# limix/CellRegMap

Measured on AMD Instinct MI355X. Metric: variant-tests/sec (interaction test), higher is better.
Workload: dtype f64

## Files before the change

cellregmap_amd/_lib.py:

```python
import ctypes
import os

import numpy as np

_HERE = os.path.dirname(os.path.abspath(__file__))
LIB_PATH = os.path.join(_HERE, "libcrm_hip.so")

c_double_p = ctypes.POINTER(ctypes.c_double)
c_int_p = ctypes.POINTER(ctypes.c_int)
c_long_p = ctypes.POINTER(ctypes.c_long)
vp = ctypes.c_void_p

SIGNATURES = {
    "crm_last_error": (ctypes.c_char_p, []),
    "crm_version": (ctypes.c_char_p, []),
    "crm_ctx_create": (ctypes.c_int, [ctypes.c_int, ctypes.POINTER(vp)]),
    "crm_ctx_destroy": (None, [vp]),
    "crm_ctx_synchronize": (ctypes.c_int, [vp]),
    "crm_ctx_trim": (ctypes.c_int, [vp]),
    "crm_background_create_qs": (ctypes.c_int, [vp, ctypes.c_long, ctypes.c_int, vp, vp, vp, vp,
                                                ctypes.POINTER(vp)]),
    "crm_background_create": (ctypes.c_int, [vp, ctypes.c_long, vp, ctypes.c_int, vp, ctypes.c_long,
                                             ctypes.c_int, vp, ctypes.c_double, ctypes.POINTER(vp)]),
    "crm_background_create_hadamard": (ctypes.c_int, [vp, ctypes.c_long, vp, ctypes.c_int, vp, ctypes.c_int, vp,
# ... 28 lines not shown
    "crm_panel_destroy": (None, [vp]),
    "crm_scan_interaction": (ctypes.c_int, [vp, vp, ctypes.c_long, ctypes.c_long] + [vp] * 13),
    "crm_scan_interaction_info": (ctypes.c_int, [vp, vp, ctypes.c_long, ctypes.c_long] + [vp] * 6),
    "crm_scan_interaction_bounds": (ctypes.c_int, [vp, vp, ctypes.c_long, ctypes.c_long] + [vp] * 8),
    "crm_scan_interaction_permuted": (ctypes.c_int, [vp, vp, ctypes.c_long, ctypes.c_long, ctypes.c_int] + [vp] * 8),
    "crm_scan_interaction_multi": (ctypes.c_int, [vp, ctypes.c_int, vp, ctypes.c_long, ctypes.c_long] + [vp] * 8),
    "crm_scan_interaction_tail": (ctypes.c_int, [vp, vp, ctypes.c_long, ctypes.c_long] + [vp] * 15),
    "crm_scan_interaction_permuted_tail": (ctypes.c_int, [vp, vp, ctypes.c_long, ctypes.c_long, ctypes.c_int] + [vp] * 10),
    "crm_scan_interaction_multi_tail": (ctypes.c_int, [vp, ctypes.c_int, vp, ctypes.c_long, ctypes.c_long] + [vp] * 10),
    "crm_scan_association": (ctypes.c_int, [vp, vp, ctypes.c_long, ctypes.c_long, ctypes.c_int, vp, vp, vp]),
    "crm_association_null_multi": (ctypes.c_int, [vp, ctypes.c_int, vp]),
    "crm_scan_association_multi": (ctypes.c_int, [vp, ctypes.c_int, vp, ctypes.c_long, ctypes.c_long, ctypes.c_int, vp, vp,
                                                  vp]),
    "crm_lmm_fit": (ctypes.c_int, [vp, ctypes.c_int, vp, vp]),
    "crm_cov_solve": (ctypes.c_int, [vp, ctypes.c_int, ctypes.c_double, ctypes.c_double, vp, ctypes.c_int, vp]),
    "crm_effects_multi": (ctypes.c_int, [vp, vp, ctypes.c_long, vp, ctypes.c_int, vp, ctypes.c_int, vp, ctypes.c_int, vp,
                                         ctypes.c_int, vp, ctypes.c_int, ctypes.c_int, vp, vp, vp, vp]),
    "crm_set_block_variants": (ctypes.c_int, [vp, ctypes.c_int]),
    "crm_set_null_fit_polish": (ctypes.c_int, [vp, ctypes.c_int]),
    "crm_set_progress_callback": (ctypes.c_int, [vp, vp, vp]),
    "crm_set_fast_rotation": (ctypes.c_int, [vp, ctypes.c_int]),
    "crm_kernel_timer_reset": (ctypes.c_int, [vp]),
    "crm_kernel_timer_read": (ctypes.c_int, [vp, c_double_p, c_long_p, c_double_p, c_double_p]),
    "crm_kernel_timer_stop": (ctypes.c_int, [vp]),
    "crm_test_set_form": (ctypes.c_int, [ctypes.c_char_p, ctypes.c_int, ctypes.c_int]),
    "crm_test_set_contraction": (ctypes.c_int, [vp, ctypes.c_int, ctypes.c_int]),
    "crm_test_set_shared_h": (ctypes.c_int, [vp, ctypes.c_int]),
    "crm_test_tail_launches": (ctypes.c_long, [vp]),
    "crm_test_spectrum_tail_launches": (ctypes.c_long, [vp]),
    "crm_test_dense_repeats": (ctypes.c_long, [vp]),
    "crm_test_donor_pair_blocks": (ctypes.c_long, [vp]),
    "crm_test_unrelated_donor_blocks": (ctypes.c_int, [vp, ctypes.POINTER(ctypes.c_long)]),
    "crm_test_gram_dma_launches": (ctypes.c_int, [vp, ctypes.POINTER(ctypes.c_long)]),
    "crm_test_tests_without_pair": (ctypes.c_long, [vp]),
    "crm_test_set_contraction_sync": (ctypes.c_int, [vp, ctypes.c_int]),
    "crm_test_sync_fallbacks": (ctypes.c_long, [vp]),
    "crm_test_overruns": (ctypes.c_long, []),
    "crm_test_live_device_bytes": (ctypes.c_long, []),
    "crm_test_set_kinship_route": (ctypes.c_int, [vp, ctypes.c_int]),
    "crm_test_check_context": (ctypes.c_int, [vp]),
    "crm_test_overrun_selftest": (ctypes.c_int, [vp]),
    "crm_test_null_fit_probe": (ctypes.c_int, [vp, ctypes.c_int, ctypes.c_double]),
    "crm_test_null_fit_probe_read": (ctypes.c_int, [vp, vp, ctypes.c_long]),
    "crm_test_contract": (ctypes.c_int, [vp, ctypes.c_long, ctypes.c_int, ctypes.c_int, vp, vp, vp,
                                         ctypes.c_int]),
    "crm_test_contract_kr": (ctypes.c_int, [vp, ctypes.c_long, ctypes.c_int, ctypes.c_int, ctypes.c_int,
                                            vp, vp, vp, vp]),
    "crm_test_contract_kr_t": (ctypes.c_int, [vp, ctypes.c_long, ctypes.c_int, ctypes.c_int, ctypes.c_int,
                                              vp, vp, vp, vp]),
    "crm_test_eigh": (ctypes.c_int, [vp, ctypes.c_int, ctypes.c_int, vp, vp, vp, ctypes.c_int, vp, vp]),
    "crm_test_eigh2": (ctypes.c_int, [vp, ctypes.c_int, ctypes.c_int, vp, vp, vp, vp, vp, ctypes.c_int, vp, vp, vp]),
    "crm_test_back_tasks": (ctypes.c_int, [ctypes.c_int, ctypes.c_long, ctypes.c_int, vp, ctypes.c_int, c_int_p]),
    "crm_test_dc_plan": (ctypes.c_int, [vp, vp, ctypes.c_int, ctypes.c_int, ctypes.c_double, c_int_p, c_double_p, vp, vp, vp,
                                        c_int_p, vp]),
    "crm_test_eigvalsh": (ctypes.c_int, [vp, ctypes.c_int, ctypes.c_int, vp, vp]),
    "crm_test_davies": (ctypes.c_int, [vp, ctypes.c_int, ctypes.c_int, vp, vp, vp, vp, vp]),
    "crm_test_tail_pvalue": (ctypes.c_int, [vp, ctypes.c_int, ctypes.c_int, vp, vp, vp, vp, vp]),
}

_lib = None


class CrmError(RuntimeError):
    pass


# ... 30 lines not shown
```

cellregmap_amd/csrc/api_core.hip:

```cpp
#include <dlfcn.h>

#include <algorithm>
#include <atomic>
#include <cstdarg>
#include <mutex>

#include <map>

#include "crm_internal.h"
#include "eigh.h"

namespace crm {

static thread_local std::string g_error;

void set_error(const char* fmt, ...) {
    char buf[1024];
    va_list ap;
    va_start(ap, fmt);
    vsnprintf(buf, sizeof buf, fmt, ap);
    va_end(ap);
    g_error = buf;
}

// ... 235 lines not shown

int crm_set_null_fit_polish(crm_ctx* c, int on) {
    return crm::guarded_on("crm_set_null_fit_polish", c, [&]() -> int {
    if (!c) return CRM_ERR_ARG;
    c->polish = on != 0;
    return CRM_OK;
    });
}

int crm_set_progress_callback(crm_ctx* c, void (*callback)(long, long, void*), void* user) {
    return crm::guarded_on("crm_set_progress_callback", c, [&]() -> int {
    if (!c) return CRM_ERR_ARG;
    if (callback) c->progress[std::this_thread::get_id()] = crm_ctx::Progress{callback, user};
    else c->progress.erase(std::this_thread::get_id());
    return CRM_OK;
    });
}

int crm_set_fast_rotation(crm_ctx* c, int on) {
    return crm::guarded_on("crm_set_fast_rotation", c, [&]() -> int {
    if (!c) return CRM_ERR_ARG;
    c->fast_T = on != 0;
    return CRM_OK;
    });
}

extern "C++" {
namespace crm {
namespace {
struct FormSlot { const char* name; int value; bool set; };
FormSlot g_forms[] = {{"gram_staged", 0, false}, {"kr_no_tail", 0, false}, {"nullfit_per_wave", 0, false}, {"kin_fold", 0, false},
                      {"eigh_one_stage", 0, false}, {"nullfit_exact", 0, false}, {"donor_pairs", 0, false},
                      {"pairs_without_kinship_term", 0, false}, {"flat_kappa_milli", 0, false}, {"chase_abort", 0, false}, {"nullfit_one_per_wave", 0, false},
                      {"kin_diag", 0, false}, {"donor_pairs_rotate", 0, false}};
std::mutex g_forms_mu;
}
int form(const char* name, int otherwise) {
    std::lock_guard<std::mutex> lock(g_forms_mu);
    for (const FormSlot& f : g_forms)
        if (strcmp(f.name, name) == 0) return f.set ? f.value : otherwise;
    return otherwise;
}
}
}

int crm_test_set_form(const char* name, int value, int reset) {
    return crm::guarded("crm_test_set_form", [&]() -> int {
    if (!name) return CRM_ERR_ARG;
    std::lock_guard<std::mutex> lock(crm::g_forms_mu);
    for (crm::FormSlot& f : crm::g_forms)
        if (strcmp(f.name, name) == 0) {
            f.value = value;
            f.set = reset == 0;
            return CRM_OK;
        }
    crm::set_error("crm_test_set_form: no kernel form is called '%s'", name);
    return CRM_ERR_ARG;
    });
}

int crm_kernel_timer_reset(crm_ctx* c) {
    return crm::guarded_on("crm_kernel_timer_reset", c, [&]() -> int {
    if (!c) return CRM_ERR_ARG;
    CRM_HIP(hipSetDevice(c->device));
    CRM_HIP(hipStreamSynchronize(c->stream));
    c->timed_used = 0;
    c->kr_flops = 0.0;
// ... 270 lines not shown
```

cellregmap_amd/csrc/crm_internal.h:

```cpp
#pragma once
#include <map>
#include <mutex>
#include <thread>
#include <type_traits>
#include <utility>

#include "crm_common.h"

namespace crm {

constexpr int CRM_DEFAULT_BLOCK = 1024;
constexpr int CRM_MAX_AUTO_BLOCK = 4096;
constexpr int CRM_MAX_RHO = 16;
constexpr int CRM_MAX_COV = 8;
constexpr int CRM_MAX_COV_WIDE = 62;
constexpr int CRM_MAX_COV_XWIDE = 128;
constexpr int CRM_MAX_K0 = 256;
constexpr int CRM_MAX_GRAM_ROWS = 288;
constexpr int DT_SUMS_LD = 136;
constexpr int BLOCK_SLACK_MAX = 4096;

struct DevBuf {
    void* ptr = nullptr;
    size_t bytes = 0;
// ... 35 lines not shown
struct crm_ctx {
    std::recursive_mutex mu;
    int device = 0;
    hipStream_t stream = nullptr;
    hipStream_t upload_stream = nullptr;
    hipEvent_t ev0 = nullptr, ev1 = nullptr;
    int block_variants = 0;
    bool fast_T = true;
    int kin_route = 1;
    bool fast_gene_rot = true;
    bool collapse = true;
    struct Progress { void (*fn)(long done, long total, void* user) = nullptr; void* user = nullptr; };
    std::map<std::thread::id, Progress> progress;
    bool progress_muted = false;
    void report(long done, long total) {
        if (progress_muted) return;
        auto it = progress.find(std::this_thread::get_id());
        if (it != progress.end() && it->second.fn) it->second.fn(done, total, it->second.user);
    }
    bool in_scan = false;
    bool polish = false;
    bool probe_on = false;
    double probe_x = 0.0;
    std::vector<double> probe_out;
    bool nullfit_exact = false;
    crm::GemmTune tune;
    crm::DevBuf sync_counters;
    unsigned* sync_timeouts_host = nullptr;
    long sync_fallbacks = 0;
    long dense_repeats = 0;
    long tail_launches = 0;
    long spectrum_tail_launches = 0;
    long donor_pair_blocks = 0;
    long unrelated_donor_blocks = 0;
    long gram_dma_launches = 0;
    long tests_without_pair = 0;
    struct ReplayBlock {
        long col0 = 0;
        int nb = 0;
        bool collapsed = false;
        std::vector<char> fit;
        crm::DevBuf T;
    };
    int replay_mode = 0;
    size_t replay_cursor = 0;
    std::vector<ReplayBlock*> replay_blocks;
    void replay_clear() {
        for (ReplayBlock* b : replay_blocks) delete b;
        replay_blocks.clear();
        replay_cursor = 0;
        replay_mode = 0;
    }
    crm::EighWork* eigh_ws = nullptr;
    bool eigh_ws_busy = false;
    bool timing = false;
    std::vector<std::pair<hipEvent_t, hipEvent_t>> timed;
    size_t timed_used = 0;
    double kr_flops = 0.0;
    crm::DevBuf ws_T, ws_A, ws_Gb, ws_Gx, ws_Gs, ws_G2, ws_GG, ws_Gt, ws_Z, ws_small, ws_probs, ws_F, ws_Gext, ws_TH, ws_AH, ws_XG;
    crm::DevBuf ws_xwide;
    crm::DevBuf ws_Tcut;
    crm::DevBuf ws_Gk, ws_S, ws_S2;
    crm::DevBuf ws_WB;
    crm::DevBuf ws_Pd;
    crm::DevBuf ws_Anone;
    std::vector<crm::DevBuf*> all_bufs() {
// ... 18 lines not shown
```

cellregmap_amd/csrc/kinship.hip:

```cpp
#include <algorithm>
#include <atomic>

#include "nullfit.h"
#include "objects.h"

using namespace crm;

namespace crm {

void jacobi_rotate(int k, double* A, double* V, int p, int q, double cs, double sn) {
    for (int r = 0; r < k; r++) {
        const double arp = A[(size_t)r * k + p], arq = A[(size_t)r * k + q];
        A[(size_t)r * k + p] = cs * arp - sn * arq;
        A[(size_t)r * k + q] = sn * arp + cs * arq;
    }
    for (int r = 0; r < k; r++) {
        const double apr = A[(size_t)p * k + r], aqr = A[(size_t)q * k + r];
        A[(size_t)p * k + r] = cs * apr - sn * aqr;
        A[(size_t)q * k + r] = sn * apr + cs * aqr;
    }
    for (int r = 0; r < k; r++) {
        const double vrp = V[(size_t)r * k + p], vrq = V[(size_t)r * k + q];
        V[(size_t)r * k + p] = cs * vrp - sn * vrq;
        V[(size_t)r * k + q] = sn * vrp + cs * vrq;
// ... 35 lines not shown
        for (long e = d + 1; e < groups; e++) {
            double s = 0.0;
            for (long q = 0; q < m; q++) s += hKd[d * m + q] * hKd[e * m + q];
            if (!(std::fabs(s) <= tol * std::sqrt(kappa[d] * kappa[e]))) return CRM_OK;
        }
    crm_ctx* ctx = bg->ctx;
    hipStream_t st = ctx->stream;
    const long ldc = round_up(KK, 128);
    if (sizeof(double) * (double)groups * KK * ldc > (double)(1ull << 30)) return CRM_OK;
    DevBuf dC, probs_dev;
    CRM_TRY(dC.ensure(sizeof(double) * (size_t)groups * KK * ldc));
    std::vector<GemmProblem> pr((size_t)groups);
    long maxlen = GEMM_BK;
    for (long d = 0; d < groups; d++) {
        GemmProblem p{};
        p.X = bg->kin_Y.as<double>() + bg->kin_row0[d] * bg->kin_ldy; p.ldx = bg->kin_ldy;
        p.Y = p.X; p.ldy = bg->kin_ldy;
        p.C = dC.as<double>() + (size_t)d * KK * ldc; p.ldc = ldc;
        p.M = KK; p.N = KK; p.cells = bg->kin_len[d];
        maxlen = std::max(maxlen, bg->kin_len[d]);
        pr[d] = p;
    }
    CRM_TRY(probs_dev.ensure(sizeof(GemmProblem) * pr.size()));
    CRM_HIP(hipMemcpyAsync(probs_dev.ptr, pr.data(), sizeof(GemmProblem) * pr.size(), hipMemcpyHostToDevice, st));
    CRM_TRY(launch_gemm_tn(ctx, probs_dev.as<GemmProblem>(), (int)groups, KK, KK, maxlen, false, 0, 1, 0));
    std::vector<double> C((size_t)groups * KK * ldc);
    CRM_HIP(hipMemcpyAsync(C.data(), dC.ptr, sizeof(double) * C.size(), hipMemcpyDeviceToHost, st));
    CRM_HIP(hipStreamSynchronize(st));
    const int k2pad = (int)round_up(k2, GEMM_BK);
    const long P = groups * k2, ldp = round_up(P, 128);
    std::vector<double> hU((size_t)groups * k2pad * 128, 0.0), hR((size_t)k1 * ldp, 0.0), hEE((size_t)k1 * k1, 0.0),
        lam((size_t)P, 0.0);
    std::vector<double> A((size_t)k2 * k2), V, w;
    for (long d = 0; d < groups; d++) {
        const double* Cd = C.data() + (size_t)d * KK * ldc;
        for (int i = 0; i < k2; i++)
            for (int j = 0; j < k2; j++) A[(size_t)i * k2 + j] = 0.5 * (Cd[i * ldc + j] + Cd[j * ldc + i]);
        jacobi_eigh(k2, A, V, w);
        double wmax = 0.0;
        for (int j = 0; j < k2; j++) wmax = std::max(wmax, w[j]);
        double* Ud = hU.data() + (size_t)d * k2pad * 128;
        for (int j = 0; j < k2; j++) {
            if (!(w[j] > (double)k2 * 2.220446049250313e-16 * wmax)) continue;
            const double sc = 1.0 / std::sqrt(w[j]);
            lam[d * k2 + j] = w[j];
            for (int q = 0; q < k2; q++) Ud[(size_t)q * 128 + j] = V[(size_t)q * k2 + j] * sc;
            for (int a = 0; a < k1; a++) {
                double s = 0.0;
                for (int q = 0; q < k2; q++) s += Ud[(size_t)q * 128 + j] * Cd[q * ldc + k2 + a];
                hR[(size_t)a * ldp + d * k2 + j] = s;
            }
        }
        for (int a = 0; a < k1; a++)
            for (int e = 0; e < k1; e++) hEE[(size_t)a * k1 + e] += Cd[(k2 + a) * ldc + k2 + e];
    }
    CRM_TRY(bg->wb_U.ensure(sizeof(double) * hU.size()));
    CRM_TRY(bg->wb_R.ensure(sizeof(double) * hR.size()));
    CRM_TRY(bg->wb_EE.ensure(sizeof(double) * hEE.size()));
    CRM_HIP(hipMemcpyAsync(bg->wb_U.ptr, hU.data(), sizeof(double) * hU.size(), hipMemcpyHostToDevice, st));
    CRM_HIP(hipMemcpyAsync(bg->wb_R.ptr, hR.data(), sizeof(double) * hR.size(), hipMemcpyHostToDevice, st));
    CRM_HIP(hipMemcpyAsync(bg->wb_EE.ptr, hEE.data(), sizeof(double) * hEE.size(), hipMemcpyHostToDevice, st));
    std::vector<std::vector<double>> s0(bg->nrho, std::vector<double>((size_t)ldp, 0.0));
    for (int i = 0; i < bg->nrho; i++) {
        for (long p = 0; p < P; p++) s0[i][p] = (1.0 - bg->rho[i]) * kappa[p / k2] * lam[p];
        CRM_TRY(bg->wb_S0[i].ensure(sizeof(double) * (size_t)ldp));
        CRM_HIP(hipMemcpyAsync(bg->wb_S0[i].ptr, s0[i].data(), sizeof(double) * (size_t)ldp, hipMemcpyHostToDevice, st));
    }
    CRM_HIP(hipStreamSynchronize(st));
    bg->wb_P = P;
    bg->wb_ldp = ldp;
    bg->wb_k2pad = k2pad;
    static std::atomic<unsigned long> wb_tables_made{0};
    bg->wb_gen = ++wb_tables_made;
    bg->kin_wb = true;
    return CRM_OK;
}

}

extern "C" {

int crm_background_set_kinship_groups(crm_background* bg, const int* group, long groups, const double* hKd, long m,
                                      const double* U, int k2) {
    return crm::guarded_on("crm_background_set_kinship_groups", bg ? bg->ctx : nullptr, [&]() -> int {
    if (!bg || !group || !hKd || !U || groups < 1 || m < 1 || k2 < 1) return CRM_ERR_ARG;
    if (bg->builder) {
        set_error("kinship groups: the background is still under construction");
        return CRM_ERR_ARG;
    }
    const long n = bg->n;
    const int k1 = (int)(bg->cols - (long)k2 * m);
    if (!bg->fast_T || !bg->H.ptr || k1 < 1 || k1 + k2 > 2 * CRM_MAX_K0 || groups > 4096) return CRM_OK;
    for (long i = 0; i < n; i++)
        if (group[i] < 0 || group[i] >= groups) {
            set_error("kinship groups: group index %d at cell %ld outside [0, %ld)", group[i], i, groups);
            return CRM_ERR_ARG;
        }
    crm_ctx* ctx = bg->ctx;
    CRM_HIP(hipSetDevice(ctx->device));
    hipStream_t st = ctx->stream;
    bg->kin = false;
    struct Undo {
// ... 131 lines not shown
```

cellregmap_amd/csrc/objects.h:

```cpp
#pragma once
#include <cmath>
#include <memory>

#include "crm_internal.h"

namespace crm {
constexpr long CELL_PAD = 128;
}

struct crm_donor_tables {
    unsigned long e0_key = 0, group_key = 0;
    unsigned long stamp = 0;
    crm::DevBuf TZ;
    crm::DevBuf Bd;
    crm::DevBuf Z2;
    crm::DevBuf Z3;
};

struct crm_background_builder;

struct crm_background {
    ~crm_background();
    crm_background_builder* builder = nullptr;
    crm_ctx* ctx = nullptr;
    long n = 0, n_pad = 0;
    int nrho = 0;
    double rho[crm::CRM_MAX_RHO] = {0};
    int r[crm::CRM_MAX_RHO] = {0};
    double ortho_defect[crm::CRM_MAX_RHO] = {0};
    long ldq = 0;
    crm::DevBuf Q0[crm::CRM_MAX_RHO];
    bool q0_ready[crm::CRM_MAX_RHO] = {false};
    crm::DevBuf Ht;
    crm::DevBuf S0[crm::CRM_MAX_RHO];
    std::vector<double> s0_max;
    bool fast_T = false;
    long ldh = 0, cols = 0;
    crm::DevBuf H;
    crm::DevBuf Mix[crm::CRM_MAX_RHO];
    bool kin = false;
    long kin_groups = 0, kin_groups_pad = 0;
    long kin_cols = 0;
    int kin_k1 = 0, kin_k2 = 0;
    long kin_rows = 0;
    std::vector<long> kin_row0, kin_len;
    crm::DevBuf kin_map;
    crm::DevBuf kin_Y;
    long kin_ldy = 128;
    crm::DevBuf kin_hKd;
    long kin_ldh = 0;
    bool kin_fold = false;
    long kin_kdim = 0;
    crm::DevBuf MixK[crm::CRM_MAX_RHO];
    bool kin_wb = false;
    long wb_P = 0, wb_ldp = 0;
    int wb_k2pad = 0;
    crm::DevBuf wb_U;
    crm::DevBuf wb_R;
    crm::DevBuf wb_EE;
    crm::DevBuf wb_S0[crm::CRM_MAX_RHO];
    unsigned long wb_gen = 0;
    static constexpr int DT_CACHE = 2;
    std::vector<crm_donor_tables*> dt_cache;
    unsigned long dt_clock = 0;
};

int crm_background_require_q0(crm_background* bg, int i);

struct crm_gene {
    crm_background* bg = nullptr;
    crm_ctx* ctx = nullptr;
    int c = 0, k0 = 0;
    long ld_yw = 0, ldw = 0, lde = 0;
    std::vector<double> W_host;
    std::vector<double> W_basis;
    crm::DevBuf yW;
    crm::DevBuf E0;
    crm::DevBuf WW, Wy;
    crm::DevBuf Wproj;
    double yy = 0.0;
    crm::DevBuf rot;
    crm::DevBuf Ep, YE, EE, idx;
    crm::DevBuf kinEp;
    crm::DevBuf kinP;
    crm::DevBuf kinUE;
    crm::DevBuf kinEE;
    crm::DevBuf wb_yW;
    unsigned long wb_gen = 0;
// ... 42 lines not shown
```

cellregmap_amd/csrc/scan.hip:

```cpp
#include <algorithm>

#include "nullfit.h"
#include "objects.h"

using namespace crm;

namespace crm {

static int ctx_cus(const crm_ctx* ctx) {
    int cus = 256;
    if (hipDeviceGetAttribute(&cus, hipDeviceAttributeMultiprocessorCount, ctx->device) != hipSuccess || cus < 1) cus = 256;
    return cus;
}

constexpr double COLLINEAR_TAU = 1e-2;

__global__ void flat_probe_fit_kernel(const crm::NullFitOut* __restrict__ fit, int count, double sign,
                                      crm::NullFitOut* __restrict__ out) {
    const int b = blockIdx.x * blockDim.x + threadIdx.x;
    if (b >= count) return;
    crm::NullFitOut f = fit[b];
    const double tiny = 2.220446049250313e-16;
    const double d = fmin(fmax(f.delta, tiny), 1.0 - tiny);
    const double x = log(d) - log1p(-d);
// ... 254 lines not shown
};

struct ScanPass {
    const std::vector<crm_gene*>& genes;
    crm_panel* panel;
    const long first, count;
    const int *idx_E, *idx_G;
    const std::vector<ScanOut>& outs;
    std::vector<long>* near_out;
    const int ng;
    crm_gene* const g0;
    crm_background* const bg;
    crm_ctx* const ctx;
    const hipStream_t st;
    const long n, np, ldq, slab;
    const int nrho, c, k0;
    ScanPlan P;
    int *d_idxE = nullptr, *d_idxG = nullptr;
    const double *d_Ep = nullptr, *d_EE = nullptr;
    crm_donor_tables* tab = nullptr;
    GemmProblem* d_probs = nullptr;
    double *dZ1 = nullptr, *dZ2 = nullptr, *dZ3 = nullptr;
    long z1_sz = 0, z2_sz = 0, z3_sz = 0;
    double *d_gg, *d_gy, *d_gW, *d_Q, *d_pv, *d_lam, *d_liu, *d_part, *d_coef, *d_thr, *d_tp, *d_tlp;
    int *d_pos, *d_ord, *d_if, *d_drop, *d_near, *d_posw, *d_tst;
    NullFitTrial* d_trial;
    NullFitOut* d_fit;
    unsigned* d_queue;
    double *wb_yW = nullptr, *wb_E1yW = nullptr, *wb_g = nullptr, *wb_Gw = nullptr, *wb_tmp = nullptr;
    std::vector<NullFitOut> h_fit = std::vector<NullFitOut>((size_t)P.BLK * ng);
    std::vector<int> h_pos = std::vector<int>((size_t)P.BLK * ng), h_ord = std::vector<int>(P.pair_cap);
    std::vector<GemmProblem> probs = std::vector<GemmProblem>(CRM_MAX_RHO + 4);
    std::vector<int> pair_of = std::vector<int>((size_t)nrho * P.BLK), h_near = std::vector<int>(P.BLK);

    ScanPass(const std::vector<crm_gene*>& genes_, crm_panel* panel_, long first_, long count_, const int* idx_E_,
             const int* idx_G_, const std::vector<ScanOut>& outs_, bool allow_collapse, std::vector<long>* near_out_)
        : genes(genes_), panel(panel_), first(first_), count(count_), idx_E(idx_E_), idx_G(idx_G_), outs(outs_),
          near_out(near_out_), ng((int)genes_.size()), g0(genes_[0]), bg(g0->bg), ctx(bg->ctx), st(ctx->stream), n(bg->n),
          np(bg->n_pad), ldq(bg->ldq), slab((long)(1 + g0->c) * bg->ldq), nrho(bg->nrho), c(g0->c), k0(g0->k0),
          P(plan_scan(genes_, panel_, idx_G_, allow_collapse, count_)) {}

    int upload(int slot, const GemmProblem* p, size_t k) {
        CRM_HIP(hipMemcpyAsync(d_probs + slot, p, sizeof(GemmProblem) * k, hipMemcpyHostToDevice, st));
        return CRM_OK;
    }
    template <class F>
    int with_records(int slot, const std::vector<GemmProblem>& kp, F&& launches) {
        CRM_TRY(upload(slot, kp.data(), kp.size()));
        CRM_TRY(launches(d_probs + slot));
        CRM_HIP(hipStreamSynchronize(st));
        return CRM_OK;
    }
    int timer_open(bool record_start) {
        if (ctx->timed_used == ctx->timed.size()) {
            hipEvent_t a, b;
            CRM_HIP(hipEventCreate(&a));
            CRM_HIP(hipEventCreate(&b));
            ctx->timed.emplace_back(a, b);
        }
        if (record_start) CRM_HIP(hipEventRecord(ctx->timed[ctx->timed_used].first, st));
        return CRM_OK;
    }
    int timer_close() {
        CRM_HIP(hipEventRecord(ctx->timed[ctx->timed_used].second, st));
        ctx->timed_used++;
        return CRM_OK;
// ... 346 lines not shown
        const long ldb = P.ldb, KK = P.KK;
        const int nb = B.nb, k1 = bg->kin_k1, k2 = bg->kin_k2;
        const long groups = bg->kin_groups, mk = bg->kin_cols;
        double* Gk = ctx->ws_Gk.as<double>();
        double* S2 = ctx->ws_S2.as<double>();
        CRM_TRY(launch_gather_rows(st, B.Gx, ldb, bg->kin_map.as<int>(), bg->kin_rows, (int)ldb, Gk, ldb));
        std::vector<GemmProblem> kp((size_t)groups + k2);
        GemmProblem p{};
        p.X = bg->kin_Y.as<double>(); p.ldx = bg->kin_ldy; p.Y = Gk; p.ldy = ldb; p.C = S2; p.ldc = ldb;
        p.M = (int)KK; p.N = nb;
        const long maxlen = donor_run_records(bg, p, KK * ldb, kp.data());
        for (int j = 0; j < k2; j++) {
            GemmProblem& q = kp[groups + j];
            q.X = bg->kin_hKd.as<double>(); q.ldx = bg->kin_ldh; q.Y = S2 + (size_t)j * ldb; q.ldy = KK * ldb;
            q.C = ctx->ws_TH.as<double>() + (size_t)(k1 + (long)j * mk) * ldb; q.ldc = ldb; q.M = (int)mk; q.N = nb;
        }
        return with_records(SLOT_KIN, kp, [&](GemmProblem* d_kp) -> int {
            CRM_TRY(launch_gemm_tn(ctx, d_kp, (int)groups, (int)KK, nb, maxlen, false, 0, 1, 0));
            CRM_TRY(launch_gemm_tn(ctx, d_kp + groups, k2, (int)mk, nb, bg->kin_groups_pad, false, 0, 1, 0));
            return launch_kin_sum_e1(st, S2, ldb, (int)KK, k2, k1, (int)groups, nb, ctx->ws_TH.as<double>(), ldb);
        });
    }

    int plain_TH(const Block& B) {
        const long ldb = P.ldb;
        GemmProblem p{};
        p.X = bg->H.as<double>(); p.ldx = bg->ldh; p.Y = B.Gx; p.ldy = ldb;
        p.C = ctx->ws_TH.as<double>(); p.ldc = ldb; p.M = (int)bg->cols; p.N = B.nb;
        CRM_TRY(upload(SLOT_ONE, &p, 1));
        CRM_TRY(launch_gemm_tn(ctx, d_probs + SLOT_ONE, 1, (int)bg->cols, B.nb, np, false, 0, P.ks_h, P.th_slab));
        return launch_reduce_splits(st, ctx->ws_TH.as<double>(), (long)bg->cols * ldb, P.ks_h, P.th_slab);
    }

    int cut_rotations(const Block& B, int& n_main) {
        const int nb = B.nb, BLK = P.BLK;
        n_main = nrho;
        const long slots = 2L * ctx_cus(ctx), mtl = (nb + GEMM_BM - 1) / GEMM_BM;
        long tiles[CRM_MAX_RHO], total = 0;
        int order[CRM_MAX_RHO];
        for (int i = 0; i < nrho; i++) { tiles[i] = mtl * ((probs[i].N + 127) / 128); total += tiles[i]; order[i] = i; }
        std::sort(order, order + nrho, [&](int a, int b) { return tiles[a] < tiles[b]; });
        const long need = total % slots;
        long acc = 0;
        int take = 0;
        while (take < nrho - 1 && acc < need) acc += tiles[order[take++]];
        if (!(total > slots && need > 0 && acc >= need && acc <= slots / 4)) return CRM_OK;
        int n_cut = 0, cut_ks = 1;
        GemmProblem cut_probs[CRM_MAX_RHO];
        double* cut_dst[CRM_MAX_RHO];
        bool is_cut[CRM_MAX_RHO] = {false};
        long cut_doubles = 0;
        for (int q = 0; q < take; q++) is_cut[order[q]] = true;
        while ((long)(cut_ks + 1) * acc <= slots && cut_ks < 16 && P.kdim / GEMM_BK / (cut_ks + 1) >= 8) cut_ks++;
        n_main = 0;
        for (int i = 0; i < nrho; i++) {
            if (!is_cut[i]) { probs[n_main++] = probs[i]; continue; }
            GemmProblem c = probs[i];
            cut_dst[n_cut] = c.C;
            c.ldc = round_up(c.N, 128);
            cut_doubles += (long)BLK * c.ldc;
            cut_probs[n_cut++] = c;
        }
        CRM_TRY(ctx->ws_Tcut.ensure(sizeof(double) * (size_t)cut_doubles * cut_ks));
        long at = 0;
        for (int q = 0; q < n_cut; q++) {
            cut_probs[q].C = ctx->ws_Tcut.as<double>() + at;
            at += (long)BLK * cut_probs[q].ldc;
        }
        const int slot = SLOT_RHO + nrho;
        CRM_TRY(upload(slot, cut_probs, n_cut));
        int cut_maxn = 1;
        for (int q = 0; q < n_cut; q++) cut_maxn = std::max(cut_maxn, cut_probs[q].N);
        CRM_TRY(launch_gemm_tn(ctx, d_probs + slot, n_cut, nb, cut_maxn, P.kdim, false, 0, cut_ks, cut_doubles));
        CRM_TRY(launch_reduce_splits(st, ctx->ws_Tcut.as<double>(), cut_doubles, cut_ks, cut_doubles));
        for (int q = 0; q < n_cut; q++)
            CRM_HIP(hipMemcpy2DAsync(cut_dst[q], sizeof(double) * P.ldT, cut_probs[q].C, sizeof(double) * cut_probs[q].ldc,
                                     sizeof(double) * cut_probs[q].N, nb, hipMemcpyDeviceToDevice, st));
        return CRM_OK;
    }

    int rotations(const Block& B) {
        const int nb = B.nb;
        if (P.folded()) CRM_TRY(fold_TH(B));
        else if (P.kin()) CRM_TRY(unfolded_TH(B));
        else if (P.fastT) CRM_TRY(plain_TH(B));
        for (int i = 0; i < nrho; i++) {
            GemmProblem p{};
            if (P.fastT) {
                p.X = ctx->ws_TH.as<double>(); p.ldx = P.ldb;
                p.Y = P.folded() ? bg->MixK[i].as<double>() : bg->Mix[i].as<double>(); p.ldy = ldq;
            } else {
                p.X = B.Gx; p.ldx = P.ldb;
                p.Y = P.collapsed() ? tab->TZ.as<double>() + (size_t)i * P.mp * ldq : bg->Q0[i].as<double>(); p.ldy = ldq;
            }
            p.C = ctx->ws_T.as<double>() + (size_t)i * P.BLK * P.ldT; p.ldc = P.ldT;
            p.M = nb; p.N = bg->r[i] > 0 ? bg->r[i] : 1;
            probs[i] = p;
        }
        int n_main = nrho;
        if (P.fastT) CRM_TRY(cut_rotations(B, n_main));
        CRM_TRY(upload(SLOT_RHO, probs.data(), n_main));
        const bool timing_T = P.wb() && ctx->timing && ctx->timed_used < 65536;
        if (timing_T) CRM_TRY(timer_open(true));
        CRM_TRY(launch_gemm_tn(ctx, d_probs + SLOT_RHO, n_main, nb, (int)ldq, P.fastT ? P.kdim : P.xrows, false, 0, 1, 0));
        if (timing_T) {
            CRM_TRY(timer_close());
            for (int q = 0; q < n_main; q++) ctx->kr_flops += 2.0 * (double)P.kdim * (double)nb * (double)probs[q].N;
        }
        return CRM_OK;
    }

    int null_fits(const Block& B) {
        const int nb = B.nb, BLK = P.BLK;
        trace_push("crm null fits");
        for (int gi = 0; gi < ng; gi++) {
            crm_gene* g = genes[gi];
            NullFitArgs fa{};
            fa.nrho = nrho; fa.c = c; fa.restricted = 1; fa.n = n; fa.polish = ctx->polish ? 1 : 0; fa.exact = (ctx->nullfit_exact || form("nullfit_exact", 0)) ? 1 : 0;
            for (int i = 0; i < nrho; i++) {
                NullFitRho& R = fa.rho[i];
                R.T = ctx->ws_T.as<double>() + (size_t)i * BLK * P.ldT; R.ldT = P.ldT;
                R.ty = g->rot.as<double>() + (long)i * slab;
                R.tW = R.ty + ldq; R.ldW = ldq;
                R.S0 = bg->S0[i].as<double>();
                R.r = bg->r[i];
            }
            fa.WW = g->WW.as<double>(); fa.Wy = g->Wy.as<double>(); fa.yy = g->yy;
            fa.gg = d_gg; fa.gy = d_gy + (size_t)gi * BLK; fa.gW = d_gW; fa.ld_gW = P.ld_gW;
            fa.g_drop = P.collapsed() ? nullptr : d_drop;
            if (c > CRM_MAX_COV_WIDE) fa.xwide = ctx->ws_xwide.as<double>();
            fa.trial = d_trial; fa.out = d_fit + (size_t)gi * BLK; fa.probe = ctx->probe_on ? 1 : 0; fa.probe_x = ctx->probe_x;
            fa.track = outs[gi].flags ? 1 : 0;
            CRM_TRY(launch_nullfit(st, fa, nb, false, d_queue));
        }
        trace_pop();
        if (ctx->probe_on) {
            std::vector<NullFitTrial> h_trial((size_t)nb * nrho);
            CRM_HIP(hipMemcpyAsync(h_trial.data(), d_trial, sizeof(NullFitTrial) * h_trial.size(), hipMemcpyDeviceToHost, st));
            CRM_HIP(hipStreamSynchronize(st));
            ctx->probe_out.assign(2 * h_trial.size(), 0.0);
            for (size_t q = 0; q < h_trial.size(); q++) {
                ctx->probe_out[2 * q] = h_trial[q].lml;
                ctx->probe_out[2 * q + 1] = h_trial[q].scale;
            }
        }
        return CRM_OK;
    }

    int replay_block(const Block& B) {
        if (ng != 1 || ctx->replay_cursor >= ctx->replay_blocks.size()) {
            set_error("scan: the replayed pass visits a block the recorded one did not");
            return CRM_ERR_INTERNAL;
        }
        crm_ctx::ReplayBlock* rb = ctx->replay_blocks[ctx->replay_cursor++];
        if (rb->col0 != B.col0 || rb->nb != B.nb || rb->collapsed != P.collapsed() || rb->fit.size() != sizeof(NullFitOut) * (size_t)B.nb) {
            set_error("scan: the replayed pass visits its blocks in another order than the recorded one");
            return CRM_ERR_INTERNAL;
        }
        CRM_HIP(hipMemcpyAsync(d_fit, rb->fit.data(), rb->fit.size(), hipMemcpyHostToDevice, st));
        if (P.wb()) CRM_TRY(fold_TH(B));
        hipLaunchKernelGGL(replay_rows_kernel, dim3((unsigned)((P.ldT + 255) / 256), B.nb), dim3(256), 0, st, ctx->ws_T.as<double>(),
                           (long)P.BLK, P.ldT, d_fit, B.nb, (int)P.ldT, rb->T.as<double>(), 1);
        CRM_HIP(hipGetLastError());
        return CRM_OK;
    }

    int woodbury_phi(const Block& B) {
        const long groups = bg->kin_groups;
        std::vector<GemmProblem> kp((size_t)groups);
        GemmProblem p{};
        p.X = ctx->ws_TH.as<double>() + (size_t)bg->kin_k1 * P.ldb; p.ldx = P.ldb; p.C = wb_g; p.ldc = P.ldwb; p.M = B.nb;
        woodbury_records(bg, p, (long)bg->kin_k2 * P.ldb, kp.data());
        CRM_TRY(with_records(SLOT_KIN, kp, [&](GemmProblem* d_kp) {
            return launch_gemm_tn(ctx, d_kp, (int)groups, B.nb, bg->kin_k2, bg->wb_k2pad, false, 0, 1, 0);
        }));
        ctx->unrelated_donor_blocks++;
        return CRM_OK;
    }

    int collect_fits(Block& B) {
        const int nb = B.nb, BLK = P.BLK;
        CRM_HIP(hipMemcpyAsync(h_fit.data(), d_fit, sizeof(NullFitOut) * (size_t)BLK * ng, hipMemcpyDeviceToHost, st));
        if (P.collapsed() && near_out) CRM_HIP(hipMemcpyAsync(h_near.data(), d_near, sizeof(int) * nb, hipMemcpyDeviceToHost, st));
        CRM_HIP(hipStreamSynchronize(st));
        if (P.collapsed() && near_out)
            for (int b = 0; b < nb; b++)
                if (h_near[b]) near_out->push_back(B.done + b);
        for (int gi = 0; gi < ng; gi++)
            for (int b = 0; b < nb; b++) {
                const int ri = h_fit[(size_t)gi * BLK + b].rho_index;
                if (ri < 0 || ri >= nrho) {
                    set_error("scan: the null fit of variant %ld (phenotype %d) did not run (grid index %d)", B.col0 + b, gi, ri);
                    return CRM_ERR_NUMERIC;
                }
            }
        if (ctx->replay_mode == 1) {
            if (ng != 1) {
                set_error("scan: the permutation replay serves one phenotype per call");
                return CRM_ERR_INTERNAL;
            }
            crm_ctx::ReplayBlock* rb = new crm_ctx::ReplayBlock();
            ctx->replay_blocks.push_back(rb);
            rb->col0 = B.col0; rb->nb = nb; rb->collapsed = P.collapsed();
            rb->fit.resize(sizeof(NullFitOut) * (size_t)nb);
            memcpy(rb->fit.data(), h_fit.data(), rb->fit.size());
            CRM_TRY(rb->T.ensure(sizeof(double) * (size_t)nb * P.ldT));
            hipLaunchKernelGGL(replay_rows_kernel, dim3((unsigned)((P.ldT + 255) / 256), nb), dim3(256), 0, st, ctx->ws_T.as<double>(),
                               (long)BLK, P.ldT, d_fit, nb, (int)P.ldT, rb->T.as<double>(), 0);
            CRM_HIP(hipGetLastError());
        }
        for (int gi = 0; gi < ng; gi++) {
            if (!outs[gi].flags) continue;
            if (B.flat_obj.empty()) B.flat_obj.assign((size_t)BLK * ng, -1.0);
            for (int b = 0; b < nb; b++) {
                const double dec = h_fit[(size_t)gi * BLK + b].decision;
                B.flat_obj[(size_t)gi * BLK + b] = dec == dec ? dec : -1.0;
            }
        }
        return CRM_OK;
    }

    SubRange sub_range(const Block& B, int b0) const {
        SubRange R;
        R.b0 = b0;
        R.nb = B.nb - b0;
        R.done = B.done + b0;
        if (ng > 1) {
            long pairs = 0;
            int take = 0;
            for (; b0 + take < B.nb; take++) {
                unsigned seen = 0;
                for (int gi = 0; gi < ng; gi++) {
                    const NullFitOut& f = h_fit[(size_t)gi * P.BLK + b0 + take];
                    if (!no_kinship_term(f)) seen |= 1u << f.rho_index;
                }
                const int here = __builtin_popcount(seen);
                if (take > 0 && pairs + here > P.pair_cap) break;
                pairs += here;
            }
            R.nb = take;
        }
        return R;
// ... 572 lines not shown
    if (ctx->polish && g0->c > CRM_MAX_COV) {
        set_error("interaction scan: the null-fit polish is only built for up to %d covariate columns", CRM_MAX_COV);
        return CRM_ERR_UNSUPPORTED;
    }
    CRM_HIP(hipSetDevice(ctx->device));
    const long n = bg->n;
    for (long i = 0; i < n; i++) {
        if ((idx_E && (idx_E[i] < 0 || idx_E[i] >= n)) || (idx_G && (idx_G[i] < 0 || idx_G[i] >= n))) {
            set_error("scan: permutation index out of range at position %ld", i);
            return CRM_ERR_ARG;
        }
    }
    if ((int)bg->s0_max.size() != bg->nrho) {
        set_error("scan: the background was not sealed");
        return CRM_ERR_INTERNAL;
    }
    ScanPass S(genes, panel, first, count, idx_E, idx_G, outs, allow_collapse, near_out);
    const ScanPlan& P = S.P;
    CRM_TRY(S.workspaces());
    CRM_TRY(S.prepare_contexts());
    CRM_TRY(S.prepare_kinship());
    CRM_TRY(S.prepare_woodbury());
    for (long done = 0; done < count; done += P.BLK) {
        Block B;
        B.done = done;
        B.col0 = first + done;
        B.nb = (int)std::min<long>(P.BLK, count - done);
        TraceRange range_block("crm scan block");
        CRM_TRY(S.copy_block(B));
        CRM_TRY(S.block_stats(B));
        if (!P.fastT && !P.collapsed()) CRM_TRY(crm_background_require_q0(bg, -1));
        if (ctx->replay_mode == 2) {
            CRM_TRY(S.replay_block(B));
        } else {
            CRM_TRY(S.rotations(B));
            CRM_TRY(S.null_fits(B));
            if (ctx->probe_on) return CRM_OK;
        }
        if (P.wb()) CRM_TRY(S.woodbury_phi(B));
        CRM_TRY(S.collect_fits(B));
        for (int b0 = 0; b0 < B.nb;) {
            const SubRange R = S.sub_range(B, b0);
            Pairs Q;
            CRM_TRY(S.select_pairs(B, R, Q));
            CRM_TRY(S.form_A(B, R, Q));
            CRM_TRY(S.side_contractions(B, R));
            CRM_TRY(S.z1_products(B, R));
            for (int gi = 0; gi < S.ng; gi++) CRM_TRY(S.gene_results(B, R, gi));
            b0 += R.nb;
        }
        ctx->report(done + B.nb, count);
    }
    return CRM_OK;
}

static int scan_core(const std::vector<crm_gene*>& genes, crm_panel* panel, long first, long count,
                     const int* idx_E, const int* idx_G, const std::vector<ScanOut>& outs) {
    std::vector<long> near;
    CRM_TRY(scan_pass(genes, panel, first, count, idx_E, idx_G, outs, true, &near));
    crm_ctx* ctx = genes[0]->ctx;
    if (near.empty() || ctx->probe_on) return CRM_OK;
    const int k0 = genes[0]->k0;
    struct Quiet {
        crm_ctx* c;
        explicit Quiet(crm_ctx* c_) : c(c_) { c->progress_muted = true; }
        ~Quiet() { c->progress_muted = false; }
    } quiet(ctx);
    ctx->dense_repeats += (long)near.size();
    if ((long)near.size() * 4 > count) {
        near.resize((size_t)count);
        for (long v = 0; v < count; v++) near[(size_t)v] = v;
    }
// ... 138 lines not shown
    o.ifault = out_ifault;
    o.liu = out_liu_pvalue;
    o.flags = out_model_flags;
    o.bound_Q = out_bound_Q;
    o.bound_p = out_bound_p;
    std::vector<ScanOut> outs{o};
    return scan_core(genes, panel, first, count, idx_E, idx_G, outs);
    });
}

long crm_test_tail_launches(const crm_ctx* ctx) { return ctx ? ctx->tail_launches : -1; }

long crm_test_spectrum_tail_launches(const crm_ctx* ctx) { return ctx ? ctx->spectrum_tail_launches : -1; }

long crm_test_dense_repeats(const crm_ctx* ctx) { return ctx ? ctx->dense_repeats : -1; }

long crm_test_donor_pair_blocks(const crm_ctx* ctx) { return ctx ? ctx->donor_pair_blocks : -1; }

int crm_test_gram_dma_launches(const crm_ctx* ctx, long* launches) {
    return crm::guarded("crm_test_gram_dma_launches", [&]() -> int {
    if (!ctx || !launches) return CRM_ERR_ARG;
    *launches = ctx->gram_dma_launches;
    return CRM_OK;
    });
}
int crm_test_unrelated_donor_blocks(const crm_ctx* ctx, long* blocks) {
    return crm::guarded("crm_test_unrelated_donor_blocks", [&]() -> int {
    if (!ctx || !blocks) return CRM_ERR_ARG;
    *blocks = ctx->unrelated_donor_blocks;
    return CRM_OK;
    });
}

long crm_test_tests_without_pair(const crm_ctx* ctx) { return ctx ? ctx->tests_without_pair : -1; }

int crm_test_set_shared_h(crm_ctx* ctx, int mode) {
    return crm::guarded_on("crm_test_set_shared_h", ctx, [&]() -> int {
    if (!ctx) return CRM_ERR_ARG;
    ctx->tune.shared_h = mode < 0 ? -1 : (mode > 0 ? 1 : 0);
    return CRM_OK;
    });
}

static int scan_multi(crm_gene* const* genes, int ngenes, crm_panel* panel, long first, long count, const int* idx_E,
                      const int* idx_G, double* out_pvalue, double* out_rho1, double* out_e2, double* out_g2,
                      double* out_eps2, double* out_Q, bool exact, double* out_logp, int* out_status) {
    if (!genes || ngenes < 1 || !panel) return CRM_ERR_ARG;
    std::vector<crm_gene*> gs(genes, genes + ngenes);
    for (crm_gene* g : gs)
        if (!g) return CRM_ERR_ARG;
    std::vector<ScanOut> outs(ngenes);
    for (int i = 0; i < ngenes; i++) {
        auto at = [&](double* base) { return base ? base + (size_t)i * count : nullptr; };
        outs[i] = ScanOut{at(out_pvalue), at(out_rho1), at(out_e2), at(out_g2), at(out_eps2), at(out_Q),
                          nullptr, nullptr, nullptr, nullptr, nullptr};
        outs[i].exact = exact;
        outs[i].logp = at(out_logp);
        outs[i].status = out_status ? out_status + (size_t)i * count : nullptr;
    }
    return scan_core(gs, panel, first, count, idx_E, idx_G, outs);
}

int crm_scan_interaction_multi(crm_gene* const* genes, int ngenes, crm_panel* panel, long first, long count,
                               const int* idx_E, const int* idx_G, double* out_pvalue, double* out_rho1,
                               double* out_e2, double* out_g2, double* out_eps2, double* out_Q) {
    return crm::guarded_on("crm_scan_interaction_multi", (genes && ngenes > 0 && genes[0]) ? genes[0]->ctx : nullptr, [&]() -> int {
// ... 19 lines not shown
```

Measured before the change: 70010.

## Skip rho=0 rotation GEMM via Woodbury positions and split ragged rotation tails

When the rho=0 background is fully captured by the Woodbury kinship factor (all eigen-directions kept), the null fit for that rho reads the Woodbury projections directly, so its rotation GEMM is dropped. Rotation GEMMs whose width leaves a small remainder past a multiple of 128 can have that remainder split off into a skinny TN kernel. A round-count model picks which of these options to apply so the main batched GEMM fills the CUs in fewer rounds. The Woodbury phi GEMM moves ahead of the rotations so the null fits can consume it, and replay no longer stores T rows in Woodbury mode. The cost is added planning logic, an extra kernel launch for the tails, and a new rho=0 path that depends on the equivalence condition holding.

After: 73140, median of 6. 1.04x the previous value.

```diff
diff --git a/cellregmap_amd/_lib.py b/cellregmap_amd/_lib.py
--- a/cellregmap_amd/_lib.py
+++ b/cellregmap_amd/_lib.py
@@ -84,6 +84,8 @@
     "crm_test_donor_pair_blocks": (ctypes.c_long, [vp]),
     "crm_test_unrelated_donor_blocks": (ctypes.c_int, [vp, ctypes.POINTER(ctypes.c_long)]),
     "crm_test_gram_dma_launches": (ctypes.c_int, [vp, ctypes.POINTER(ctypes.c_long)]),
+    "crm_test_rho0_position_blocks": (ctypes.c_int, [vp, ctypes.POINTER(ctypes.c_long)]),
+    "crm_test_rotation_tail_launches": (ctypes.c_int, [vp, ctypes.POINTER(ctypes.c_long)]),
     "crm_test_tests_without_pair": (ctypes.c_long, [vp]),
     "crm_test_set_contraction_sync": (ctypes.c_int, [vp, ctypes.c_int]),
     "crm_test_sync_fallbacks": (ctypes.c_long, [vp]),
diff --git a/cellregmap_amd/csrc/api_core.hip b/cellregmap_amd/csrc/api_core.hip
--- a/cellregmap_amd/csrc/api_core.hip
+++ b/cellregmap_amd/csrc/api_core.hip
@@ -291,7 +291,8 @@
 FormSlot g_forms[] = {{"gram_staged", 0, false}, {"kr_no_tail", 0, false}, {"nullfit_per_wave", 0, false}, {"kin_fold", 0, false},
                       {"eigh_one_stage", 0, false}, {"nullfit_exact", 0, false}, {"donor_pairs", 0, false},
                       {"pairs_without_kinship_term", 0, false}, {"flat_kappa_milli", 0, false}, {"chase_abort", 0, false}, {"nullfit_one_per_wave", 0, false},
-                      {"kin_diag", 0, false}, {"donor_pairs_rotate", 0, false}};
+                      {"kin_diag", 0, false}, {"donor_pairs_rotate", 0, false}, {"rho0_positions", 0, false},
+                      {"rotation_tails", 0, false}};
 std::mutex g_forms_mu;
 }
 int form(const char* name, int otherwise) {
diff --git a/cellregmap_amd/csrc/crm_internal.h b/cellregmap_amd/csrc/crm_internal.h
--- a/cellregmap_amd/csrc/crm_internal.h
+++ b/cellregmap_amd/csrc/crm_internal.h
@@ -91,6 +91,8 @@
     long tail_launches = 0;
     long spectrum_tail_launches = 0;
     long donor_pair_blocks = 0;
+    long rotation_tail_launches = 0;
+    long rho0_position_blocks = 0;
     long unrelated_donor_blocks = 0;
     long gram_dma_launches = 0;
     long tests_without_pair = 0;
diff --git a/cellregmap_amd/csrc/kinship.hip b/cellregmap_amd/csrc/kinship.hip
--- a/cellregmap_amd/csrc/kinship.hip
+++ b/cellregmap_amd/csrc/kinship.hip
@@ -91,6 +91,7 @@
     std::vector<double> hU((size_t)groups * k2pad * 128, 0.0), hR((size_t)k1 * ldp, 0.0), hEE((size_t)k1 * k1, 0.0),
         lam((size_t)P, 0.0);
     std::vector<double> A((size_t)k2 * k2), V, w;
+    long kept = 0;
     for (long d = 0; d < groups; d++) {
         const double* Cd = C.data() + (size_t)d * KK * ldc;
         for (int i = 0; i < k2; i++)
@@ -103,6 +104,7 @@
             if (!(w[j] > (double)k2 * 2.220446049250313e-16 * wmax)) continue;
             const double sc = 1.0 / std::sqrt(w[j]);
             lam[d * k2 + j] = w[j];
+            kept++;
             for (int q = 0; q < k2; q++) Ud[(size_t)q * 128 + j] = V[(size_t)q * k2 + j] * sc;
             for (int a = 0; a < k1; a++) {
                 double s = 0.0;
@@ -127,6 +129,7 @@
     }
     CRM_HIP(hipStreamSynchronize(st));
     bg->wb_P = P;
+    bg->wb_kept = kept;
     bg->wb_ldp = ldp;
     bg->wb_k2pad = k2pad;
     static std::atomic<unsigned long> wb_tables_made{0};
diff --git a/cellregmap_amd/csrc/objects.h b/cellregmap_amd/csrc/objects.h
--- a/cellregmap_amd/csrc/objects.h
+++ b/cellregmap_amd/csrc/objects.h
@@ -54,6 +54,7 @@
     crm::DevBuf MixK[crm::CRM_MAX_RHO];
     bool kin_wb = false;
     long wb_P = 0, wb_ldp = 0;
+    long wb_kept = 0;
     int wb_k2pad = 0;
     crm::DevBuf wb_U;
     crm::DevBuf wb_R;
diff --git a/cellregmap_amd/csrc/scan.hip b/cellregmap_amd/csrc/scan.hip
--- a/cellregmap_amd/csrc/scan.hip
+++ b/cellregmap_amd/csrc/scan.hip
@@ -310,6 +310,9 @@
     std::vector<int> h_pos = std::vector<int>((size_t)P.BLK * ng), h_ord = std::vector<int>(P.pair_cap);
     std::vector<GemmProblem> probs = std::vector<GemmProblem>(CRM_MAX_RHO + 4);
     std::vector<int> pair_of = std::vector<int>((size_t)nrho * P.BLK), h_near = std::vector<int>(P.BLK);
+    bool rho0_pos[CRM_MAX_RHO] = {false};
+    std::vector<GemmProblem> rot_tails;
+    std::vector<GemmProblem> phi_recs;
 
     ScanPass(const std::vector<crm_gene*>& genes_, crm_panel* panel_, long first_, long count_, const int* idx_E_,
              const int* idx_G_, const std::vector<ScanOut>& outs_, bool allow_collapse, std::vector<long>* near_out_)
@@ -722,28 +725,37 @@
         return launch_reduce_splits(st, ctx->ws_TH.as<double>(), (long)bg->cols * ldb, P.ks_h, P.th_slab);
     }
 
-    int cut_rotations(const Block& B, int& n_main) {
-        const int nb = B.nb, BLK = P.BLK;
-        n_main = nrho;
+    bool cut_choice(int nb, int cnt, const int* N, bool* is_cut, long& acc, long& rounds) const {
         const long slots = 2L * ctx_cus(ctx), mtl = (nb + GEMM_BM - 1) / GEMM_BM;
         long tiles[CRM_MAX_RHO], total = 0;
         int order[CRM_MAX_RHO];
-        for (int i = 0; i < nrho; i++) { tiles[i] = mtl * ((probs[i].N + 127) / 128); total += tiles[i]; order[i] = i; }
-        std::sort(order, order + nrho, [&](int a, int b) { return tiles[a] < tiles[b]; });
+        for (int i = 0; i < cnt; i++) { tiles[i] = mtl * ((N[i] + 127) / 128); total += tiles[i]; order[i] = i; }
+        std::sort(order, order + cnt, [&](int a, int b) { return tiles[a] < tiles[b]; });
         const long need = total % slots;
-        long acc = 0;
+        acc = 0;
         int take = 0;
-        while (take < nrho - 1 && acc < need) acc += tiles[order[take++]];
-        if (!(total > slots && need > 0 && acc >= need && acc <= slots / 4)) return CRM_OK;
+        while (take < cnt - 1 && acc < need) acc += tiles[order[take++]];
+        const bool cut = total > slots && need > 0 && acc >= need && acc <= slots / 4;
+        rounds = ((cut ? total - acc : total) + slots - 1) / slots;
+        for (int q = 0; q < take && cut; q++) is_cut[order[q]] = true;
+        return cut;
+    }
+    int cut_rotations(const Block& B, int n_list, int& n_main) {
+        const int nb = B.nb, BLK = P.BLK;
+        n_main = n_list;
+        const long slots = 2L * ctx_cus(ctx);
+        int widths[CRM_MAX_RHO];
+        bool is_cut[CRM_MAX_RHO] = {false};
+        long acc = 0, rounds = 0;
+        for (int i = 0; i < n_list; i++) widths[i] = probs[i].N;
+        if (!cut_choice(nb, n_list, widths, is_cut, acc, rounds)) return CRM_OK;
         int n_cut = 0, cut_ks = 1;
         GemmProblem cut_probs[CRM_MAX_RHO];
         double* cut_dst[CRM_MAX_RHO];
-        bool is_cut[CRM_MAX_RHO] = {false};
         long cut_doubles = 0;
-        for (int q = 0; q < take; q++) is_cut[order[q]] = true;
         while ((long)(cut_ks + 1) * acc <= slots && cut_ks < 16 && P.kdim / GEMM_BK / (cut_ks + 1) >= 8) cut_ks++;
         n_main = 0;
-        for (int i = 0; i < nrho; i++) {
+        for (int i = 0; i < n_list; i++) {
             if (!is_cut[i]) { probs[n_main++] = probs[i]; continue; }
             GemmProblem c = probs[i];
             cut_dst[n_cut] = c.C;
@@ -757,7 +769,7 @@
             cut_probs[q].C = ctx->ws_Tcut.as<double>() + at;
             at += (long)BLK * cut_probs[q].ldc;
         }
-        const int slot = SLOT_RHO + nrho;
+        const int slot = SLOT_RHO + n_main;
         CRM_TRY(upload(slot, cut_probs, n_cut));
         int cut_maxn = 1;
         for (int q = 0; q < n_cut; q++) cut_maxn = std::max(cut_maxn, cut_probs[q].N);
@@ -774,6 +786,8 @@
         if (P.folded()) CRM_TRY(fold_TH(B));
         else if (P.kin()) CRM_TRY(unfolded_TH(B));
         else if (P.fastT) CRM_TRY(plain_TH(B));
+        if (P.wb()) CRM_TRY(woodbury_phi(B));
+        GemmProblem all[CRM_MAX_RHO];
         for (int i = 0; i < nrho; i++) {
             GemmProblem p{};
             if (P.fastT) {
@@ -785,10 +799,12 @@
             }
             p.C = ctx->ws_T.as<double>() + (size_t)i * P.BLK * P.ldT; p.ldc = P.ldT;
             p.M = nb; p.N = bg->r[i] > 0 ? bg->r[i] : 1;
-            probs[i] = p;
-        }
-        int n_main = nrho;
-        if (P.fastT) CRM_TRY(cut_rotations(B, n_main));
+            all[i] = p;
+        }
+        const int n_list = plan_rotations(B, all);
+        if (n_list == 0) return CRM_OK;
+        int n_main = n_list;
+        if (P.fastT) CRM_TRY(cut_rotations(B, n_list, n_main));
         CRM_TRY(upload(SLOT_RHO, probs.data(), n_main));
         const bool timing_T = P.wb() && ctx->timing && ctx->timed_used < 65536;
         if (timing_T) CRM_TRY(timer_open(true));
@@ -797,7 +813,59 @@
             CRM_TRY(timer_close());
             for (int q = 0; q < n_main; q++) ctx->kr_flops += 2.0 * (double)P.kdim * (double)nb * (double)probs[q].N;
         }
-        return CRM_OK;
+        if (!rot_tails.empty()) {
+            CRM_TRY(upload(SLOT_RHO + n_list, rot_tails.data(), rot_tails.size()));
+            CRM_TRY(launch_skinny_tn(st, d_probs + SLOT_RHO + n_list, (int)rot_tails.size(), nb, P.kdim));
+            ctx->rotation_tail_launches++;
+        }
+        return CRM_OK;
+    }
+
+    int plan_rotations(const Block& B, const GemmProblem* all) {
+        const int mode0 = P.fastT && P.wb() ? form("rho0_positions", 1) : 0;
+        const int modeT = P.fastT && P.kin() && !form("kr_no_tail", 0) ? form("rotation_tails", 1) : 0;
+        bool cand[CRM_MAX_RHO] = {false};
+        int rem[CRM_MAX_RHO] = {0}, n_cand = 0, n_rem = 0;
+        for (int i = 0; i < nrho; i++) {
+            const GemmProblem& p = all[i];
+            cand[i] = mode0 > 0 && bg->rho[i] == 0.0 && bg->r[i] > 0 && bg->wb_kept == bg->r[i];
+            const int m = p.N % 128;
+            if (modeT > 0 && p.N >= 1024 && m > 0 && m <= 16 && p.ldx % 2 == 0 && (reinterpret_cast<uintptr_t>(p.X) & 15) == 0) rem[i] = m;
+            n_cand += cand[i] ? 1 : 0;
+        }
+        for (int i = 0; i < nrho; i++) n_rem += rem[i] > 0 ? 1 : 0;
+        auto rounds = [&](bool drop, bool tails) {
+            int widths[CRM_MAX_RHO], cnt = 0;
+            bool is_cut[CRM_MAX_RHO] = {false};
+            long acc = 0, r = 0;
+            for (int i = 0; i < nrho; i++)
+                if (!(drop && cand[i])) widths[cnt++] = all[i].N - (tails ? rem[i] : 0);
+            if (cnt > 0) cut_choice(B.nb, cnt, widths, is_cut, acc, r);
+            return r;
+        };
+        const bool can0 = n_cand > 0, canT = n_rem > 0, force0 = mode0 >= 2 && can0, forceT = modeT >= 2 && canT;
+        bool drop = force0, tails = forceT;
+        long best = rounds(drop, tails);
+        for (int pick = 1; pick < 4; pick++) {
+            const bool d = force0 || (can0 && (pick & 1)), t = forceT || (canT && (pick & 2));
+            const long r = rounds(d, t);
+            if (r < best) { best = r; drop = d; tails = t; }
+        }
+        rot_tails.clear();
+        int n_list = 0;
+        for (int i = 0; i < nrho; i++) {
+            rho0_pos[i] = drop && cand[i];
+            if (rho0_pos[i]) continue;
+            GemmProblem p = all[i];
+            if (tails && rem[i] > 0) {
+                GemmProblem t = p;
+                p.N -= rem[i];
+                t.Y = p.Y + p.N; t.C = p.C + p.N; t.N = rem[i];
+                rot_tails.push_back(t);
+            }
+            probs[n_list++] = p;
+        }
+        return n_list;
     }
 
     int null_fits(const Block& B) {
@@ -814,6 +882,13 @@
                 R.tW = R.ty + ldq; R.ldW = ldq;
                 R.S0 = bg->S0[i].as<double>();
                 R.r = bg->r[i];
+                if (rho0_pos[i]) {
+                    R.T = wb_g; R.ldT = P.ldwb;
+                    R.ty = wb_yW + (size_t)gi * (1 + c) * P.ldwb;
+                    R.tW = R.ty + P.ldwb; R.ldW = P.ldwb;
+                    R.S0 = bg->wb_S0[i].as<double>();
+                    R.r = (int)bg->wb_P;
+                }
             }
             fa.WW = g->WW.as<double>(); fa.Wy = g->Wy.as<double>(); fa.yy = g->yy;
             fa.gg = d_gg; fa.gy = d_gy + (size_t)gi * BLK; fa.gW = d_gW; fa.ld_gW = P.ld_gW;
@@ -824,6 +899,7 @@
             CRM_TRY(launch_nullfit(st, fa, nb, false, d_queue));
         }
         trace_pop();
+        if (std::find(rho0_pos, rho0_pos + nrho, true) != rho0_pos + nrho) ctx->rho0_position_blocks++;
         if (ctx->probe_on) {
             std::vector<NullFitTrial> h_trial((size_t)nb * nrho);
             CRM_HIP(hipMemcpyAsync(h_trial.data(), d_trial, sizeof(NullFitTrial) * h_trial.size(), hipMemcpyDeviceToHost, st));
@@ -848,7 +924,7 @@
             return CRM_ERR_INTERNAL;
         }
         CRM_HIP(hipMemcpyAsync(d_fit, rb->fit.data(), rb->fit.size(), hipMemcpyHostToDevice, st));
-        if (P.wb()) CRM_TRY(fold_TH(B));
+        if (P.wb()) return fold_TH(B);
         hipLaunchKernelGGL(replay_rows_kernel, dim3((unsigned)((P.ldT + 255) / 256), B.nb), dim3(256), 0, st, ctx->ws_T.as<double>(),
                            (long)P.BLK, P.ldT, d_fit, B.nb, (int)P.ldT, rb->T.as<double>(), 1);
         CRM_HIP(hipGetLastError());
@@ -857,15 +933,12 @@
 
     int woodbury_phi(const Block& B) {
         const long groups = bg->kin_groups;
-        std::vector<GemmProblem> kp((size_t)groups);
+        phi_recs.resize((size_t)groups);
         GemmProblem p{};
         p.X = ctx->ws_TH.as<double>() + (size_t)bg->kin_k1 * P.ldb; p.ldx = P.ldb; p.C = wb_g; p.ldc = P.ldwb; p.M = B.nb;
-        woodbury_records(bg, p, (long)bg->kin_k2 * P.ldb, kp.data());
-        CRM_TRY(with_records(SLOT_KIN, kp, [&](GemmProblem* d_kp) {
-            return launch_gemm_tn(ctx, d_kp, (int)groups, B.nb, bg->kin_k2, bg->wb_k2pad, false, 0, 1, 0);
-        }));
-        ctx->unrelated_donor_blocks++;
-        return CRM_OK;
+        woodbury_records(bg, p, (long)bg->kin_k2 * P.ldb, phi_recs.data());
+        CRM_TRY(upload(SLOT_KIN, phi_recs.data(), phi_recs.size()));
+        return launch_gemm_tn(ctx, d_probs + SLOT_KIN, (int)groups, B.nb, bg->kin_k2, bg->wb_k2pad, false, 0, 1, 0);
     }
 
     int collect_fits(Block& B) {
@@ -894,10 +967,12 @@
             rb->col0 = B.col0; rb->nb = nb; rb->collapsed = P.collapsed();
             rb->fit.resize(sizeof(NullFitOut) * (size_t)nb);
             memcpy(rb->fit.data(), h_fit.data(), rb->fit.size());
-            CRM_TRY(rb->T.ensure(sizeof(double) * (size_t)nb * P.ldT));
-            hipLaunchKernelGGL(replay_rows_kernel, dim3((unsigned)((P.ldT + 255) / 256), nb), dim3(256), 0, st, ctx->ws_T.as<double>(),
-                               (long)BLK, P.ldT, d_fit, nb, (int)P.ldT, rb->T.as<double>(), 0);
-            CRM_HIP(hipGetLastError());
+            if (!P.wb()) {
+                CRM_TRY(rb->T.ensure(sizeof(double) * (size_t)nb * P.ldT));
+                hipLaunchKernelGGL(replay_rows_kernel, dim3((unsigned)((P.ldT + 255) / 256), nb), dim3(256), 0, st, ctx->ws_T.as<double>(),
+                                   (long)BLK, P.ldT, d_fit, nb, (int)P.ldT, rb->T.as<double>(), 0);
+                CRM_HIP(hipGetLastError());
+            }
         }
         for (int gi = 0; gi < ng; gi++) {
             if (!outs[gi].flags) continue;
@@ -1536,12 +1611,13 @@
         if (!P.fastT && !P.collapsed()) CRM_TRY(crm_background_require_q0(bg, -1));
         if (ctx->replay_mode == 2) {
             CRM_TRY(S.replay_block(B));
+            if (P.wb()) CRM_TRY(S.woodbury_phi(B));
         } else {
             CRM_TRY(S.rotations(B));
             CRM_TRY(S.null_fits(B));
             if (ctx->probe_on) return CRM_OK;
         }
-        if (P.wb()) CRM_TRY(S.woodbury_phi(B));
+        if (P.wb()) ctx->unrelated_donor_blocks++;
         CRM_TRY(S.collect_fits(B));
         for (int b0 = 0; b0 < B.nb;) {
             const SubRange R = S.sub_range(B, b0);
@@ -1746,6 +1822,21 @@
     });
 }
 
+int crm_test_rho0_position_blocks(const crm_ctx* ctx, long* blocks) {
+    return crm::guarded("crm_test_rho0_position_blocks", [&]() -> int {
+    if (!ctx || !blocks) return CRM_ERR_ARG;
+    *blocks = ctx->rho0_position_blocks;
+    return CRM_OK;
+    });
+}
+int crm_test_rotation_tail_launches(const crm_ctx* ctx, long* launches) {
+    return crm::guarded("crm_test_rotation_tail_launches", [&]() -> int {
+    if (!ctx || !launches) return CRM_ERR_ARG;
+    *launches = ctx->rotation_tail_launches;
+    return CRM_OK;
+    });
+}
+
 long crm_test_tests_without_pair(const crm_ctx* ctx) { return ctx ? ctx->tests_without_pair : -1; }
 
 int crm_test_set_shared_h(crm_ctx* ctx, int mode) {
```
